# aouyang1/go-muse

Hardware: AMD Instinct MI355X
Metric: series-pairs XCorr/sec at N=4096, 1M-series batch; achieved HBM GB/s (higher is better)
Workload: dtype f64

## Files before the change

go-muse_amd/binding.py:

```python
import ctypes
import os

import numpy as np

from . import build as _build

_i32 = ctypes.c_int32
_i64 = ctypes.c_int64
_f64 = ctypes.c_double
_vp = ctypes.c_void_p
_dp = ctypes.POINTER(ctypes.c_double)
_i32p = ctypes.POINTER(ctypes.c_int32)
_i64p = ctypes.POINTER(ctypes.c_int64)

MUSE_OK = 0
MUSE_ERR_INVALID = -1
MUSE_ERR_LENGTH = -2
MUSE_ERR_ZERO_STD = -3
MUSE_ERR_NO_DEVICE = -4
MUSE_ERR_HIP = -5
MUSE_ERR_UNSUPPORTED = -6
MUSE_ERR_NOMEM = -7
MUSE_ERR_EMPTY = -8
MUSE_LAG_WINDOW_MAX = 63
# ... 116 lines not shown
                                                        _i64p, _i32p, _dp, _i32p, _dp]),
    "muse_test_many_lag_range_plan": (ctypes.c_int, [_i32, _i32, _i32, _i32, _i32, _i32p]),
    "muse_test_window_many_plan_rows": (ctypes.c_int, [_i32, _i32, _i32p, _i32p, _i32p, _i32p, _i32p, _i32p]),
    "muse_batch_run_many": (ctypes.c_int, [ctypes.POINTER(_vp), _i32, _i32p, _i32, _i32, _i32, _f64, _i32, _i32,
                                           _i64p, _i32p, _dp, _i32p, _dp]),
    "muse_batch_free": (ctypes.c_int, [_vp]),
    "muse_xcorr_with_x": (ctypes.c_int, [_vp, _dp, _dp, _i32, _i32, _dp, _i32p, _dp, _i32p]),
    "muse_xcorr": (ctypes.c_int, [_vp, _dp, _i32, _dp, _i32, _i32, _i32, _dp, _i32p, _dp, _i32p]),
    "muse_xcorr_groups": (ctypes.c_int, [_vp, _vp, _i32, _i32, _i32p, _dp, _i32p, _dp]),
    "muse_xcorr_batch": (ctypes.c_int, [_vp, _dp, _dp, _i64, _i32, _i32, _i32, _i32, _i32p, _dp, _i32p, _dp]),
    "muse_ctx_set_spectrum_cache": (ctypes.c_int, [_vp, _i32]),
    "muse_group_spectrum_cache": (ctypes.c_int, [_vp, _i64p, _i64p]),
    "muse_group_drop_spectrum_cache": (ctypes.c_int, [_vp]),
    "muse_test_spectrum_cache_limits": (ctypes.c_int, [_vp, _i64, _i64]),
    "muse_test_spectrum_cache_reader": (ctypes.c_int, [_vp, _i32]),
    "muse_test_spectrum_cache_policy": (ctypes.c_int, [_i64, _i32, _i32, _i32, _i64, _i64, _i64, _i32p, _i64p, _i64p]),
    "muse_test_batch_redo_pairs": (ctypes.c_int, [_vp, _i64p, _i64, _i64p]),
    "muse_next_pow2": (_i64, [_f64]),
}


class MuseError(RuntimeError):
    def __init__(self, status, message):
        super().__init__("muse_hip status %d: %s" % (status, message))
        self.status = status
        self.message = message


_lib = None

# ... 46 lines not shown
```

go-muse_amd/csrc/capi_batch.hip:

```cpp
#include "capi_internal.h"
#include "xcorr_huge.h"

using namespace muse;


int ilog2(int64_t n)
{
    int l = 0;
    while (((int64_t)1 << l) < n)
        l++;
    return l;
}

int build_spectrum(muse_ctx *ctx, const double *ref_host, int N, int n, int normalize, double x_scale,
                          double xc_scale, double2 *X, double2 *xc, float2 *xcf, double *xs, int *zero_std)
{
    double *dref = nullptr;
    int *dstat = nullptr;
    double2 *dscr = nullptr;
    HIP_TRY(dmalloc(ctx, &dref, (size_t)N * sizeof(double)));
    hipError_t e = dmalloc(ctx, &dstat, sizeof(int));
    if (e == hipSuccess && n > GENERIC_LDS_MAX_N)
        e = dmalloc(ctx, &dscr, (size_t)n * sizeof(double2));
    if (e == hipSuccess)
// ... 74 lines not shown
        return fail(MUSE_ERR_INVALID, "series length 1 has no sample standard deviation");
    const int64_t n = muse_next_pow2((double)N);
    if (n > HUGE_MAX_N)
        return fail(MUSE_ERR_UNSUPPORTED, "FFT length %lld > %d is not built", (long long)n, HUGE_MAX_N);
    const bool huge = n > GENERIC_MAX_N;
    muse_batch *b = new (std::nothrow) muse_batch();
    if (!b)
        return fail(MUSE_ERR_NOMEM, "host allocation failed");
    b->ctx = ctx;
    b->g = g;
    g->refs.fetch_add(1);
    ctx->refs.fetch_add(1);
    b->N = N;
    b->n = (int32_t)n;
    b->logn = ilog2(n);
    hipError_t e = dmalloc(ctx, &b->ovf_count, 2 * sizeof(int));
    if (e == hipSuccess && !huge)
        e = ensure_gscratch(ctx, n);
    muse_spectrum *sp = new (std::nothrow) muse_spectrum();
    if (!sp)
        e = hipErrorOutOfMemory;
    b->sp = sp;
    if (e == hipSuccess)
        e = dmalloc(ctx, &sp->X, (size_t)(n / 2 + 1) * sizeof(double2));
    if (huge) {
        if (e == hipSuccess)
            e = dmalloc(ctx, &sp->xcp, (size_t)n * sizeof(double2));
        if (e != hipSuccess) {
            muse_batch_free(b);
            return fail(MUSE_ERR_NOMEM, "hipMalloc failed: %s", hipGetErrorString(e));
        }
// ... 97 lines not shown
    if (rc)
        return rc;
    muse_batch *b = new (std::nothrow) muse_batch();
    if (!b)
        return fail(MUSE_ERR_NOMEM, "host allocation failed");
    b->ctx = ctx;
    b->g = g;
    g->refs.fetch_add(1);
    ctx->refs.fetch_add(1);
    b->N = src->N;
    b->n = src->n;
    b->logn = src->logn;
    b->sp = src->sp;
    b->sp->refs.fetch_add(1);
    adopt_spectrum(b);
    hipError_t e = dmalloc(ctx, &b->ovf_count, 2 * sizeof(int));
    if (e != hipSuccess) {
        muse_batch_free(b);
        return fail(MUSE_ERR_NOMEM, "hipMalloc failed: %s", hipGetErrorString(e));
    }
    *out = b;
    return MUSE_OK;
}

extern "C" int muse_batch_fft_len(muse_batch *b, int32_t *n)
{
    if (!b || !n)
        return fail(MUSE_ERR_INVALID, "NULL argument");
    *n = b->n;
    return MUSE_OK;
}
// ... 262 lines not shown
    ctx->zc_min_rows.store(min_rows < 0 ? ZC_MIN_ROWS : min_rows);
    ctx->zc_budget.store(budget_bytes < 0 ? -1 : budget_bytes);
    return MUSE_OK;
}

extern "C" int muse_test_spectrum_cache_reader(muse_ctx *ctx, int32_t reader)
{
    if (!ctx)
        return fail(MUSE_ERR_INVALID, "NULL context");
    if (reader != 0 && reader != 1)
        return fail(MUSE_ERR_INVALID, "spectrum cache reader %d (0 = two workgroups per CU, 1 = four)", (int)reader);
    ctx->zc_reader.store(reader);
    return MUSE_OK;
}

extern "C" int muse_test_spectrum_cache_policy(int64_t rows, int32_t N, int32_t f32, int32_t mode, int64_t min_rows,
                                               int64_t free_bytes, int64_t budget_bytes, int32_t *decision,
                                               int64_t *rows_cached, int64_t *bytes)
{
    if (!decision || !rows_cached || !bytes)
        return fail(MUSE_ERR_INVALID, "NULL output");
    *decision = spectrum_cache_policy(rows, N, f32 != 0, mode, min_rows < 0 ? ZC_MIN_ROWS : min_rows, free_bytes,
                                      budget_bytes < 0 ? -1 : budget_bytes, rows_cached, bytes);
    return MUSE_OK;
}

extern "C" int muse_test_batch_redo_pairs(muse_batch *b, int64_t *pairs, int64_t cap, int64_t *count)
{
    if (!b || !count || cap < 0 || (cap > 0 && !pairs))
        return fail(MUSE_ERR_INVALID, "bad redo-list arguments");
// ... 92 lines not shown
    const bool allow_spectrum_cache = pass.allow_spectrum_cache;
    const SlideFuse *slide = pass.slide;
    if (slide) {
        if (variant != KERNEL_R16_FOLD || allow_spectrum_cache)
            return fail(MUSE_ERR_INVALID, "the fused slide runs in the default n = 4096 kernel, off the rows");
        p.slide_tails = slide->tails;
        p.slide_k = slide->k;
    }
    if (variant == KERNEL_GENERIC && b->n <= GENERIC_LDS_MAX_N)
        p.gscratch = nullptr;
    LaunchTimer timer(ctx, false, st);
    LaunchTimer redo_timer(ctx, true, st);
    if (variant == KERNEL_R16_FOLD) {
        HIP_TRY(b->ovf_list.ensure(ctx, 2 * p.npairs, st));
        p.ovf_count = b->ovf_count;
        p.work_counter = b->ovf_count + 1;
        p.ovf_list = b->ovf_list.p;
        HIP_TRY(hipMemsetAsync(b->ovf_count, 0, 2 * sizeof(int), st));
        ZcPlan plan;
        std::unique_lock<std::mutex> zc_lock(b->g->ready_mu, std::defer_lock);
        if (allow_spectrum_cache && !mask && spectrum_cache_candidate(b, variant)) {
            zc_lock.lock();
            rc = plan_spectrum_cache(b, plan);
            if (rc)
                return rc;
            if (!plan.use)
                zc_lock.unlock();
        }
        HIP_TRY(timer.begin());
        if (plan.use) {
            bool launched = false;
            const auto next_launch = [&]() {
                const hipError_t e = launched ? hipMemsetAsync(b->ovf_count + 1, 0, sizeof(int), st) : hipSuccess;
                launched = true;
                return e;
            };
            const bool occ4_reader = ctx->zc_reader.load() == 1;
            for (const auto &sg : plan.readers) {
                FusedParams r = p;
                r.npairs = sg.pairs;
                HIP_TRY(next_launch());
                HIP_TRY(launch_cached(r, SpectrumCacheArgs{sg.zc(), sg.zstat(), sg.pair0, sg.pairs}, ctx->num_cus, st, occ4_reader));
            }
            if (plan.tail_pair0 < p.npairs) {
                FusedParams w = p;
                w.npairs = p.npairs - plan.tail_pair0;
                HIP_TRY(next_launch());
                HIP_TRY(launch_cache_fill(w, SpectrumCacheArgs{plan.tail_zpairs ? plan.tail_seg.zc() : nullptr,
                                                               plan.tail_zpairs ? plan.tail_seg.zstat() : nullptr,
                                                               plan.tail_pair0, plan.tail_zpairs}, ctx->num_cus, st));
            }
            zc_lock.unlock();
        } else {
            HIP_TRY(launch_fused(p, variant, ctx->num_cus, st));
        }
        HIP_TRY(timer.end());
        FusedParams q = p;
        q.slide_tails = nullptr;
        q.slide_k = 0;
        q.pair_list = b->ovf_list.p;
        q.pair_count = b->ovf_count;
        q.dense_total = ctx->variant == 0 ? p.npairs : 0;
        q.npairs = std::min<long long>(p.npairs, (long long)ctx->num_cus * 3);
        HIP_TRY(redo_timer.begin());
        HIP_TRY(launch_fused(q, KERNEL_R16_OCC3, ctx->num_cus, st));
        HIP_TRY(redo_timer.end());
        if (p.npairs >= 1024 && !(b->handoff_host && b->handoff_M == M && b->handoff_rewrites == b->g->rewrites)) {
            if (!b->handoff_host)
// ... 72 lines not shown
                 window_wide(b->g->rows, b->g->stride) ? "true" : "false");
    } else if (b->n > GENERIC_MAX_N) {
        snprintf(k, sizeof(k), "huge_rows<false>");
    } else {
        const KernelChoice kc = choose_kernel(b, (b->g->M + 1) / 2);
        switch (kc.error ? -1 : kc.variant) {
        case KERNEL_R16_FOLD: {
            bool cached = false;
            if (spectrum_cache_candidate(b, kc.variant)) {
                std::lock_guard<std::mutex> lock(b->g->ready_mu);
                int64_t rc_ = 0, by_ = 0;
                cached = b->g->zc_state == muse_group::ZC_VALID && b->g->zc_rewrites == b->g->rewrites && b->g->zc_rows > 0 &&
                         spectrum_cache_policy(b->g->M, b->N, false, b->ctx->zc_mode.load(), b->ctx->zc_min_rows.load(), 0, 0, &rc_, &by_) != ZC_POLICY_NONE;
            }
            if (cached)
                snprintf(k, sizeof(k), "xcorr_cached_n4096%s<%s>", b->ctx->zc_reader.load() == 1 ? "_occ4" : "", padded);
            else
                snprintf(k, sizeof(k), "xcorr_fused_n4096_fold<false, %s, %s>", padded, f32);
            break;
        }
        case KERNEL_R16_OCC3: snprintf(k, sizeof(k), "xcorr_fused_n4096_occ4"); break;
        case KERNEL_SMALL: snprintf(k, sizeof(k), "xcorr_fused_small<%d, %s, false, %s>", b->logn, padded, f32); break;
        case KERNEL_LONG: snprintf(k, sizeof(k), "xcorr_fused_long<%d, %s, false>", b->logn, padded); break;
        case KERNEL_STOCKHAM: snprintf(k, sizeof(k), b->n >= 8192 ? "xcorr_fused_stk_4step" : "xcorr_fused_stockham"); break;
        case KERNEL_REAL_SPLIT: snprintf(k, sizeof(k), "xcorr_fused_real32k_split<%s>", padded); break;
        case KERNEL_REAL: snprintf(k, sizeof(k), "xcorr_fused_real%dk<%s>", b->n / 1024, padded); break;
        default: break;
        }
    }
    snprintf(name, (size_t)cap, "%s", k);
    return MUSE_OK;
// ... 14 lines not shown
        dfree(c, b->sp->xcf);
        dfree(c, b->sp->xs);
        dfree(c, b->sp->c1);
        delete b->sp;
    }
    if (b->small_out) {
        std::lock_guard<std::mutex> lock(c->small_mu);
        c->small_free.emplace_back(b->small_out, b->small_cap);
    }
    dfree(c, b->ovf_count);
    hfree(c, b->handoff_host);
    hfree(c, b->refine_host);
    hfree(c, b->err_host);
    dfree(c, b->err_dev);
    b->ovf_list.release(c);
    b->mv.release(c);
    b->lag.release(c);
    b->gid_dev.release(c);
    b->gkey.release(c);
    b->gfirst.release(c);
    b->gwin.release(c);
    b->rec.release(c);
    b->selkey.release(c);
    b->cand.release(c);
    b->cnt.release(c);
    b->cand_host.release(c);
    b->cnt_host.release(c);
    b->rec_host.release(c);
    b->key_host.release(c);
    b->scr_flags.release(c);
// ... 17 lines not shown
```

go-muse_amd/csrc/capi_internal.h:

```cpp
#pragma once
#include <hip/hip_runtime.h>

#include <algorithm>
#include <atomic>
#include <mutex>
#include <cmath>
#include <cstdarg>
#include <cstdio>
#include <cstdlib>
#include <cstring>
#include <ctime>
#include <limits>
#include <map>
#include <new>
#include <string>
#include <unordered_map>
#include <utility>
#include <vector>

#include "muse_hip.h"
#include "muse_hip_test.h"
#include "xcorr_kernels.h"

using namespace muse;
// ... 92 lines not shown
    MemPool dev_pool, host_pool;
    HugeWork huge;
    int huge_batch_mb = 0;
    std::mutex huge_mu;
    std::mutex small_mu;
    std::vector<std::pair<unsigned char *, int>> small_free;
    unsigned long long small_token = 0;
    std::mutex timing_mu;
    std::atomic<bool> rows_always_copy{false};
    std::vector<void *> rows_slots;
    std::mutex rows_mu;
    std::atomic<int> zc_mode{1};
    std::atomic<int64_t> zc_min_rows{ZC_MIN_ROWS};
    std::atomic<int64_t> zc_budget{-1};
    std::atomic<int> zc_reader{0};
    std::atomic<int> win_rows_slices{0};
    std::atomic<bool> in_window_force{false};
    std::atomic<int> slide_in_window_force{0};
    std::atomic<bool> gather_nt{false};
    std::atomic<int> refs{1};
};

struct muse_group {
    std::atomic<int> refs{1};
    muse_ctx *ctx = nullptr;
    double *rows = nullptr;
    float *rows32 = nullptr;
    bool f32 = false;
    size_t elem() const { return f32 ? sizeof(float) : sizeof(double); }
    void *base() const { return f32 ? (void *)rows32 : (void *)rows; }
// ... 74 lines not shown
        OWN = 0,
        PLAIN = MUSE_IN_WINDOW_PLAIN, MFMA = MUSE_IN_WINDOW_MFMA, MASKED = MUSE_IN_WINDOW_MASKED
    };
    static constexpr int32_t MANY = -1;
    Kind kind = OWN;
    LagRange window{0, 0, 0};
    int32_t variant = 0;
    int32_t tiles = 0;
    int32_t slide = 0;
    static ScoreOrigin packed(int32_t tiles) { return ScoreOrigin{PACKED, LagRange{0, 0, 0}, 0, tiles}; }
    static ScoreOrigin in_window(int32_t path, const LagRange &w, int32_t variant = 0) { return ScoreOrigin{(Kind)path, w, variant}; }
    int32_t in_window_path() const { return kind > OWN ? (int32_t)kind : 0; }
    int32_t mfma_tiles() const { return (window.rows() + 15) / 16; }
};

struct muse_batch {
    muse_ctx *ctx = nullptr;
    muse_group *g = nullptr;
    hipStream_t own_stream = nullptr;
    hipStream_t stream() const { return own_stream ? own_stream : ctx->stream; }
    int32_t N = 0, n = 0, logn = 0;
    muse_spectrum *sp = nullptr;
    double *c1 = nullptr;
    double2 *X = nullptr, *xc = nullptr;
    double2 *xcp = nullptr;
    double2 *xcw = nullptr;
    float2 *xcf = nullptr;
    double *xs = nullptr;
    int *ovf_count = nullptr;
    int *handoff_host = nullptr;
    int64_t handoff_M = -1;
    uint64_t handoff_rewrites = 0;
    PoolBuf<long long> ovf_list;
    PoolBuf<double> mv;
    PoolBuf<int> lag;
    unsigned char *small_out = nullptr;
    int small_cap = 0;
    PoolBuf<int> gid_dev;
    std::vector<int32_t> gid_host;
    bool gid_valid = false;
    PoolBuf<unsigned long long> gkey;
    PoolBuf<long long> gfirst, gwin;
    GroupWork gw() const { return GroupWork{gkey.p, gfirst.p, gwin.p}; }
    PoolBuf<muse_record> rec;
    PoolBuf<unsigned long long> selkey;
    PoolBuf<muse_record> cand;
    PoolBuf<int> cnt;
    HostBuf<muse_record> cand_host;
// ... 181 lines not shown
```

go-muse_amd/csrc/capi_many.hip:

```cpp
#include "capi_internal.h"

using namespace muse;


int upload_many_tab(muse_ctx *ctx, std::vector<void *> &tab, bool zscratch)
{
    if (zscratch)
        HIP_TRY(ctx->zscratch.ensure(ctx, (int64_t)ctx->num_cus * 4 * 4096, ctx->stream));
    HIP_TRY(ctx->many_tab.ensure(ctx, (int64_t)tab.size(), ctx->stream));
    HIP_TRY(hipStreamSynchronize(ctx->stream));
    ctx->many_host.swap(tab);
    HIP_TRY(hipMemcpyAsync(ctx->many_tab.p, ctx->many_host.data(), ctx->many_host.size() * sizeof(void *),
                           hipMemcpyHostToDevice, ctx->stream));
    return MUSE_OK;
}

extern "C" int muse_batch_read_scores(muse_batch *b, int32_t *lag, double *mv)
{
    if (!b)
        return fail(MUSE_ERR_INVALID, "NULL batch");
    int rc = use_device(b->ctx);
    if (rc)
        return rc;
    const int64_t M = b->g->M;
// ... 85 lines not shown
    if (rc)
        return rc;
    void **const t = ctx->many_tab.p;
    FusedParams p = base_params(b0);
    p.R = R;
    p.xcp_many = (const double2 *const *)t;
    p.mv_many = (double *const *)(t + R);
    p.lag_many = (int *const *)(t + 2 * R);
    p.c1_many = (const double *const *)(t + 3 * R);
    p.zscratch = ctx->zscratch.p;
    p.zslots = (int)(ctx->zscratch.cap / 4096);
    if (mask)
        set_window(p, *mask);
    HIP_TRY(b0->ovf_list.ensure(ctx, 2 * p.npairs, b0->stream()));
    p.ovf_count = b0->ovf_count;
    p.work_counter = b0->ovf_count + 1;
    p.ovf_list = b0->ovf_list.p;
    std::unique_lock<std::mutex> scratch_lock(ctx->stage_mu, std::defer_lock);
    if (long_n || real_n) {
        scratch_lock.lock();
        p.gscratch = ctx->gscratch.p;
        p.gscratch_slices = (long long)(ctx->gscratch.cap / b0->n);
    }
    LaunchTimer timer(ctx);
    HIP_TRY(hipMemsetAsync(b0->ovf_count, 0, 2 * sizeof(int), ctx->stream));
    HIP_TRY(timer.begin());
    if (small_n) {
        HIP_TRY(launch_fused_small(p, ctx->num_cus, ctx->stream));
    } else if (real_n) {
        p.gsmall = ctx->gsmall[4];
        HIP_TRY(launch_fused_real_split(p, ctx->num_cus, ctx->stream));
    } else if (long_n)
        HIP_TRY(launch_fused_long(p, ctx->num_cus, ctx->stream));
    else
        HIP_TRY(launch_fused_multi(p, ctx->num_cus, ctx->stream));
    HIP_TRY(timer.end());
    const bool redo = !small_n && !real_n;
    LaunchTimer redo_timer(ctx, true);
    if (redo)
        HIP_TRY(redo_timer.begin());
// ... 88 lines not shown
```

go-muse_amd/csrc/capi_rows.hip:

```cpp
#include "capi_internal.h"

using namespace muse;

namespace {
constexpr size_t ROWS_GUARD = 8192;
constexpr size_t ROWS_SLOT_MIN_ELEMS = 1u << 16;
constexpr size_t ROWS_SLOT_MAX_ELEMS = 1u << 24;
constexpr size_t ROWS_ZERO_COPY_BYTES = 256u << 10;
constexpr size_t ROWS_SLOT_KEEP_ELEMS = 1u << 20;
constexpr int ROWS_SLOTS_KEPT = 16;
}

struct RowsSlot {
    muse_group g;
    muse_batch b;
    double *dev = nullptr;
    double *host = nullptr;
    double *host_dev = nullptr;
    size_t cap_elems = 0;
    SingleGroupOut *out = nullptr;
    hipEvent_t done = nullptr;
    hipStream_t stream = nullptr;
    PoolBuf<double> win_e, win_pw, win_slabs;
    uint64_t win_serial = 0;
// ... 15 lines not shown
        (void)hipStreamSynchronize(s->stream);
    dfree(ctx, s->dev);
    if (s->host)
        hfree(ctx, s->host - ROWS_GUARD);
    if (s->out)
        (void)hipHostFree(s->out);
    if (s->done)
        (void)hipEventDestroy(s->done);
    s->g.hstats.release(ctx);
    s->b.mv.release(ctx);
    s->b.lag.release(ctx);
    s->win_e.release(ctx);
    s->win_pw.release(ctx);
    s->win_slabs.release(ctx);
    s->b.ovf_list.release(ctx);
    dfree(ctx, s->b.ovf_count);
    hfree(ctx, s->b.handoff_host);
    if (s->stream)
        (void)hipStreamDestroy(s->stream);
    delete s;
}

void rows_slots_free(muse_ctx *ctx)
{
    for (void *p : ctx->rows_slots)
        slot_destroy((RowsSlot *)p);
    ctx->rows_slots.clear();
}

static int slot_reserve(RowsSlot *s, size_t elems)
// ... 38 lines not shown
        }
    }
    if (!s) {
        s = new (std::nothrow) RowsSlot();
        if (!s)
            return fail(MUSE_ERR_NOMEM, "host allocation failed");
        s->g.ctx = ctx;
        s->b.ctx = ctx;
        s->b.g = &s->g;
        hipError_t e = hipHostMalloc((void **)&s->out, sizeof(SingleGroupOut), hipHostMallocCoherent | hipHostMallocMapped);
        if (e == hipSuccess)
            e = hipEventCreateWithFlags(&s->done, hipEventDisableTiming);
        if (e == hipSuccess)
            e = hipStreamCreateWithFlags(&s->stream, hipStreamNonBlocking);
        if (e == hipSuccess)
            e = dmalloc(ctx, &s->b.ovf_count, 2 * sizeof(int));
        if (e != hipSuccess) {
            slot_destroy(s);
            return fail(MUSE_ERR_HIP, "slot set-up failed: %s", hipGetErrorString(e));
        }
    }
    int rc = slot_reserve(s, elems);
    if (rc) {
        slot_destroy(s);
        return rc;
    }
    *out = s;
    return MUSE_OK;
}

static void slot_return(muse_ctx *ctx, RowsSlot *s)
// ... 399 lines not shown
```

go-muse_amd/csrc/n4096_pair_device.h:

```cpp
#pragma once
#include "foldk_device.h"

namespace muse {

namespace foldk {

#if defined(__HIP_DEVICE_COMPILE__)
typedef d2v __attribute__((address_space(1))) *zc_out_ptr;
typedef double __attribute__((address_space(1))) *zstat_out_ptr;
typedef const double __attribute__((address_space(4))) *zstat_in_ptr;
#endif

struct PairThread {
    int t, lane, wave;
    double invN, invNm1;
};
template <bool PADDED>
__device__ __forceinline__ PairThread pair_prologue(const FusedParams &p, double2 *g2s, double *prev_row, const int rec_stride)
{
    PairThread th;
    th.t = threadIdx.x;
    th.lane = th.t & 63;
    th.wave = __builtin_amdgcn_readfirstlane(th.t >> 6);
    th.invN = PADDED ? p.invN : 1.0 / 4096.0;
// ... 123 lines not shown
    const zstat_in_ptr sp = (zstat_in_ptr)(unsigned long long)(zstat + rel * ZC_STAT);
#pragma unroll
    for (int k = 0; k < 10; k++)
        st[k] = sp[k];
#endif
}
__device__ __forceinline__ void publish_pair_stats(double *rec, const double (&st)[10], const int t, const long long rA, const bool hasB)
{
    if (t == 0) {
#pragma unroll
        for (int k = 0; k < 10; k++)
            rec[24 + k] = st[k];
        rec[34] = (double)rA;
        rec[35] = hasB ? 1.0 : 0.0;
    }
}

struct NoTap {
    static constexpr long long first = 0;
    __device__ __forceinline__ void operator()(const double2 (&)[16], const double *, double, double, long long, int) const {}
};

template <bool TIMING, bool PADDED, bool F32, bool WIN, bool SLIDE, typename Tap>
__device__ __forceinline__ void pair_loop_from_rows(const FusedParams &p, const Tap tap)
{
    __shared__ double2 xbuf[OCC_XBUF];
    __shared__ double2 g2s[128];
    __shared__ double red[2 * REC];
    __shared__ int next_s[2];
    const PairThread th = pair_prologue<PADDED>(p, g2s, red + 34, REC);
// ... 106 lines not shown
```

go-muse_amd/csrc/xcorr_kernels.h:

```cpp
#pragma once
#include <hip/hip_runtime.h>
#include <stdint.h>
#include <type_traits>

#include "muse_hip.h"

namespace muse {

enum { KERNEL_GENERIC = 0, KERNEL_R16_OCC3 = 6, KERNEL_STOCKHAM = 10, KERNEL_R16_FOLD = 11, KERNEL_SMALL = 12, KERNEL_LONG = 13, KERNEL_REAL = 14, KERNEL_REAL_SPLIT = 15 };

struct FusedParams {
    const double *rows;
    const float *rows32;
    long long M;
    long long stride;
    long long npairs;
    int N;
    int n;
    int logn;
    int normalize_y;
    const double2 *xc;
    const double2 *tw1;
    const double2 *tw2;
    const double2 *xcp;
// ... 35 lines not shown
    int scr_need_sign;
    int *ovf_count;
    int *work_counter;
    long long *ovf_list;
    const long long *pair_list;
    const int *pair_count;
    long long dense_total;
    long long gscratch_slices;
    const double *xrows;
    long long xstride;
    int Nx;
    double invN, invNm1;
    int win, win_lpos, win_lneg;
    const void *slide_tails;
    int slide_k;
};
inline FusedParams with_reciprocals(FusedParams p)
{
    p.invN = 1.0 / (double)p.N;
    p.invNm1 = 1.0 / (double)(p.N - 1);
    return p;
}
inline bool window_bounds_ok(const FusedParams &p)
{
    return !p.win || (p.win_lpos >= 0 && p.win_lneg >= 0 && p.win_lpos <= 2048 && p.win_lneg <= 2047);
}
template <typename F>
inline void with_bools(F f)
{
    f();
}
// ... 206 lines not shown
```

go-muse_amd/csrc/xcorr_r16_cached.hip:

```cpp
#include <hip/hip_runtime.h>
#include <stdint.h>
#include <algorithm>

#include "n4096_pair_device.h"

namespace muse {

struct CacheTap {
    const SpectrumCacheArgs c;
    const long long first;
    __device__ __forceinline__ void operator()(const double2 (&v)[16], const double *rec, const double s1a, const double s1b,
                                               const long long rel, const int t) const
    {
#if defined(__HIP_DEVICE_COMPILE__)
        if (rel < c.zpairs) {
            const foldk::zc_out_ptr zo = (foldk::zc_out_ptr)(unsigned long long)(c.zc + rel * 4096) + t;
#pragma unroll
            for (int i = 0; i < 16; i++)
                __builtin_nontemporal_store(occ4::d2v{v[i].x, v[i].y}, zo + 256 * i);
            if (t < 10) {
                const foldk::zstat_out_ptr so = (foldk::zstat_out_ptr)(unsigned long long)(c.zstat + rel * ZC_STAT);
                so[t] = t < 8 ? rec[24 + t] : (t == 8 ? s1a : s1b);
            }
        }
// ... 15 lines not shown
        switch (s) {
        case 0: return foldk::G3Derived::sq(foldk::G3Derived::sq(w8));
        case 1: return foldk::G3Derived::sq(w8);
        case 2: return w8;
        case 3: return make_double2(H * (w8.x + w8.y), H * (w8.y - w8.x));
        case 4: return w16;
        case 5: return foldk::G3Derived::mulc(w16, fold::C16_1, fold::S16_1);
        case 6: return make_double2(H * (w16.x + w16.y), H * (w16.y - w16.x));
        default: return foldk::G3Derived::mulc(w16, fold::S16_1, fold::C16_1);
        }
    }
};

constexpr int ZC_CLAIM = 2;

template <bool PADDED>
__global__ __launch_bounds__(OCC_THREADS, 2) void xcorr_cached_n4096(const FusedParams p, const SpectrumCacheArgs c)
{
    using namespace occ4;
    using namespace fold;
    using namespace foldk;
    __shared__ double2 xbuf[OCC_XBUF_FULL];
    __shared__ double2 g2s[128];
    __shared__ double red[2 * REC];
    __shared__ int next_s[2];
    const PairThread th = pair_prologue<PADDED>(p, g2s, red + 34, REC);
    const int t = th.t, lane = th.lane, wave = th.wave;
    const double invN = th.invN, invNm1 = th.invNm1;
    double2 *const xw = xbuf + 1088 * wave;
    const long long first = c.pair0, total = c.pair0 + p.npairs;
    constexpr bool AHEAD = !PADDED;
    constexpr int ch = ZC_CLAIM;

    if (t == 0)
        next_s[1] = (int)gridDim.x + atomicAdd(p.work_counter, 1);
    d2v zn[16];
    request_z(zn, c, first + (long long)ch * blockIdx.x, t);
    double2 xf[16];
#pragma unroll
    for (int j = 0; j < 16; j++)
        xf[j] = XcFetch{p.xcp, t}(j);
    G3Lazy g3{G3Fetch{p.g3b, t}(2), G3Fetch{p.g3b, t}(4)};
    __syncthreads();

    int parity = 0, cpar = 0;
    long long pair = first + (long long)ch * blockIdx.x;
    long long cbeg = pair, cend = pair + ch < total ? pair + ch : total;
    long long nchunk = first + (long long)ch * __builtin_amdgcn_readfirstlane(next_s[1]), after = 0;
    while (pair < total) {
        const bool claiming = pair == cbeg;
        const long long nextpair = pair + 1 < cend ? pair + 1 : nchunk;
        const long long rA = 2 * pair;
        const bool hasB = rA + 1 < p.M;
        double *const rec = red + REC * parity;
        const double *const prec = red + REC * (parity ^ 1);
        double st[10];
        load_pair_stats(st, c.zstat, pair - first);
        double2 v[16];
#pragma unroll
        for (int i = 0; i < 16; i++)
            v[i] = make_double2(zn[i].x, zn[i].y);
        xc_stage1_pre(v, xf);
        int claim = 0;
#pragma unroll
        for (int i = 0; i < 16; i += 4)
            asm volatile("" : "+v"(v[i].x), "+v"(v[i].y), "+v"(v[i + 1].x), "+v"(v[i + 1].y), "+v"(v[i + 2].x), "+v"(v[i + 2].y), "+v"(v[i + 3].x), "+v"(v[i + 3].y));
#if defined(__HIP_DEVICE_COMPILE__)
        if (claiming && t == 0) {
            unsigned long long wc = (unsigned long long)p.work_counter;
            asm volatile("" : "+v"(wc));
            claim = __hip_atomic_fetch_add((int __attribute__((address_space(1))) *)wc, 1, __ATOMIC_RELAXED, __HIP_MEMORY_SCOPE_AGENT);
        }
#endif
        const long long nxt = nextpair < total ? nextpair : first;
        if (AHEAD) {
            fence();
            request_z(zn, c, nxt, t);
            fence();
        }
        asm volatile("" : "+v"(g3.w8.x), "+v"(g3.w8.y), "+v"(g3.w16.x), "+v"(g3.w16.y));
        dft16_rn_s234(v);
        exchange_local_full<0>(v, xw, t);
        gdft16_nr(v, G2Fetch{g2s, t & 15});
        if (claiming && t == 0)
            next_s[cpar] = (int)gridDim.x + claim;
        exchange_cross_full<1, 1>(v, xbuf, t);
        lds_barrier();
        finalize_pair(prec, wave, lane == 0, invN, invNm1, p);
        publish_pair_stats(rec, st, t, rA, hasB);
        if (claiming) {
            after = first + (long long)ch * __builtin_amdgcn_readfirstlane(next_s[cpar]);
            cpar ^= 1;
        }
        gdft16_nr_l2(v, g3);
        if (PADDED)
            correct_padded<16>(v, p.c1, t, st[8] * invN, st[9] * invN, [&]() __attribute__((always_inline)) {
                request_z(zn, c, nxt, t);
                fence();
            });
        wave_argmax_store(v, wave, lane, rec + 6 * wave);
        parity ^= 1;
        if (pair + 1 < cend) {
            pair++;
        } else {
            pair = cbeg = nchunk;
            cend = pair + ch < total ? pair + ch : total;
            nchunk = after;
        }
    }
    lds_barrier();
    finalize_pair(red + REC * (parity ^ 1), t, true, invN, invNm1, p);
}

template <bool PADDED>
__global__ __launch_bounds__(OCC_THREADS, 4) void xcorr_cached_n4096_occ4(const FusedParams p, const SpectrumCacheArgs c)
{
    using namespace occ4;
    using namespace fold;
    using namespace foldk;
    __shared__ double2 xbuf[OCC_XBUF];
    __shared__ double2 g2s[128];
    __shared__ double red[2 * REC];
    __shared__ int next_s[2];
    const PairThread th = pair_prologue<PADDED>(p, g2s, red + 34, REC);
    const int t = th.t, lane = th.lane, wave = th.wave;
    const double invN = th.invN, invNm1 = th.invNm1;
// ... 50 lines not shown
}

hipError_t launch_cache_fill(const FusedParams &p_in, const SpectrumCacheArgs &c, int num_cus, hipStream_t stream)
{
    const FusedParams p = with_reciprocals(p_in);
    if (!cache_launch_ok(p, c) || c.zpairs < 0 || c.zpairs > p.npairs || (c.zpairs > 0 && (!c.zc || !c.zstat)) ||
        2 * (c.pair0 + c.zpairs) > p.M)
        return hipErrorInvalidValue;
    const dim3 g((unsigned)std::min<long long>(p.npairs, (long long)num_cus * 4)), b(OCC_THREADS);
    with_bools([&](auto padded) { hipLaunchKernelGGL((xcorr_cache_fill_n4096<decltype(padded)::value>), g, b, 0, stream, p, c); }, p.N < 4096);
    return hipGetLastError();
}

hipError_t launch_cached(const FusedParams &p_in, const SpectrumCacheArgs &c, int num_cus, hipStream_t stream, bool occ4)
{
    const FusedParams p = with_reciprocals(p_in);
    if (!cache_launch_ok(p, c) || !c.zc || !c.zstat || c.zpairs < p.npairs || 2 * (c.pair0 + p.npairs) > p.M)
        return hipErrorInvalidValue;
    const dim3 g((unsigned)(occ4 ? std::min<long long>(p.npairs, (long long)num_cus * 4)
                                 : std::min<long long>((p.npairs + ZC_CLAIM - 1) / ZC_CLAIM, (long long)num_cus * 2))), b(OCC_THREADS);
    with_bools([&](auto four, auto padded) {
        if (decltype(four)::value)
            hipLaunchKernelGGL((xcorr_cached_n4096_occ4<decltype(padded)::value>), g, b, 0, stream, p, c);
        else
            hipLaunchKernelGGL((xcorr_cached_n4096<decltype(padded)::value>), g, b, 0, stream, p, c);
    }, occ4, p.N < 4096);
    return hipGetLastError();
}

}

#undef MUSE_CONSUME_ROWS
```

go-muse_amd/muse.py:

```python
import ctypes
import math
import sys
import threading
import uuid
import weakref

import numpy as np

from . import binding as B
from .binding import MuseError

DefaultLabel = "uid"

SignFilter_POS = 1
SignFilter_NEG = -1
SignFilter_ANY = 0


class Engine:

    def __init__(self, device=0):
        self._h = ctypes.c_void_p()
        B.check(B.load().muse_ctx_create(int(device), ctypes.byref(self._h)))
        self.device = int(device)
# ... 33 lines not shown

    def set_screening(self, enable, min_rows=None):
        B.check(B.load().muse_ctx_set_screening(self._h, (int(min_rows) if min_rows and min_rows > 1 else 1) if enable else 0))

    def set_screen_bound_scale(self, scale):
        B.check(B.load().muse_test_set_screen_bound_scale(self._h, float(scale)))

    def set_spectrum_cache(self, on):
        B.check(B.load().muse_ctx_set_spectrum_cache(self._h, 1 if on else 0))

    def spectrum_cache_limits(self, min_rows=-1, budget_bytes=-1):
        B.check(B.load().muse_test_spectrum_cache_limits(self._h, int(min_rows), int(budget_bytes)))

    def spectrum_cache_reader(self, reader=0):
        B.check(B.load().muse_test_spectrum_cache_reader(self._h, int(reader)))

    def trim(self):
        B.check(B.load().muse_ctx_trim(self._h))

    def pool_stats(self):
        v = [ctypes.c_int64(0) for _ in range(4)]
        B.check(B.load().muse_test_pool_stats(self._h, *[ctypes.byref(x) for x in v]))
        return tuple(int(x.value) for x in v)

    def xcorr_repeat(self, repeat):
        B.check(B.load().muse_test_xcorr_repeat(self._h, int(repeat)))

    def huge_batch_mb(self, megabytes):
        B.check(B.load().muse_test_huge_batch_mb(self._h, int(megabytes)))

# ... 1435 lines not shown
```

Baseline: 160.5 million.

## Add sharded work-counter hand-out for cached reader and pad counter word

Adds an optional sharded pair hand-out for the cached N=4096 reader kernel. It is tunable through test hooks: several atomic counters spaced a configurable stride apart, each workgroup starting at a home shard and moving on when that shard runs out, plus a configurable claim size. The default work counter is also moved to a separate 256-byte-offset word, so it no longer shares a cache line with the overflow count. The aim is to cut atomic contention and false sharing on a single counter, at the cost of extra memsets and a more complex claim path.

```diff
diff --git a/go-muse_amd/binding.py b/go-muse_amd/binding.py
--- a/go-muse_amd/binding.py
+++ b/go-muse_amd/binding.py
@@ -154,6 +154,8 @@
     "muse_group_drop_spectrum_cache": (ctypes.c_int, [_vp]),
     "muse_test_spectrum_cache_limits": (ctypes.c_int, [_vp, _i64, _i64]),
     "muse_test_spectrum_cache_reader": (ctypes.c_int, [_vp, _i32]),
+    "muse_test_handout": (ctypes.c_int, [_vp, _i32, _i32]),
+    "muse_test_handout_stride": (ctypes.c_int, [_vp, _i32]),
     "muse_test_spectrum_cache_policy": (ctypes.c_int, [_i64, _i32, _i32, _i32, _i64, _i64, _i64, _i32p, _i64p, _i64p]),
     "muse_test_batch_redo_pairs": (ctypes.c_int, [_vp, _i64p, _i64, _i64p]),
     "muse_next_pow2": (_i64, [_f64]),
diff --git a/go-muse_amd/csrc/capi_batch.hip b/go-muse_amd/csrc/capi_batch.hip
--- a/go-muse_amd/csrc/capi_batch.hip
+++ b/go-muse_amd/csrc/capi_batch.hip
@@ -112,7 +112,7 @@
     b->N = N;
     b->n = (int32_t)n;
     b->logn = ilog2(n);
-    hipError_t e = dmalloc(ctx, &b->ovf_count, 2 * sizeof(int));
+    hipError_t e = dmalloc(ctx, &b->ovf_count, OVF_COUNT_INTS * sizeof(int));
     if (e == hipSuccess && !huge)
         e = ensure_gscratch(ctx, n);
     muse_spectrum *sp = new (std::nothrow) muse_spectrum();
@@ -240,7 +240,7 @@
     b->sp = src->sp;
     b->sp->refs.fetch_add(1);
     adopt_spectrum(b);
-    hipError_t e = dmalloc(ctx, &b->ovf_count, 2 * sizeof(int));
+    hipError_t e = dmalloc(ctx, &b->ovf_count, OVF_COUNT_INTS * sizeof(int));
     if (e != hipSuccess) {
         muse_batch_free(b);
         return fail(MUSE_ERR_NOMEM, "hipMalloc failed: %s", hipGetErrorString(e));
@@ -533,6 +533,32 @@
     return MUSE_OK;
 }
 
+extern "C" int muse_test_handout(muse_ctx *ctx, int32_t shards, int32_t claim)
+{
+    if (!ctx)
+        return fail(MUSE_ERR_INVALID, "NULL context");
+    if (shards < 0 || shards > HANDOUT_MAX_SHARDS || claim < 0 || claim > HANDOUT_MAX_CLAIM)
+        return fail(MUSE_ERR_INVALID, "pair hand-out of %d counters, %d pairs per add (0 = the default; at most %d and %d)", (int)shards,
+                    (int)claim, HANDOUT_MAX_SHARDS, HANDOUT_MAX_CLAIM);
+    ctx->hand_shards.store(shards);
+    ctx->hand_claim.store(claim);
+    return MUSE_OK;
+}
+
+extern "C" int muse_test_handout_stride(muse_ctx *ctx, int32_t bytes)
+{
+    if (!ctx)
+        return fail(MUSE_ERR_INVALID, "NULL context");
+    int shift = 0;
+    while (bytes > 0 && (4 << shift) < bytes)
+        shift++;
+    if (bytes < 0 || (bytes > 0 && ((4 << shift) != bytes || shift < 4 || shift > HANDOUT_SHIFT_MAX)))
+        return fail(MUSE_ERR_INVALID, "hand-out counters %d bytes apart (0 = the default; a power of two, 64 ... %d)", (int)bytes,
+                    4 << HANDOUT_SHIFT_MAX);
+    ctx->hand_shift.store(shift);
+    return MUSE_OK;
+}
+
 extern "C" int muse_test_spectrum_cache_policy(int64_t rows, int32_t N, int32_t f32, int32_t mode, int64_t min_rows,
                                                int64_t free_bytes, int64_t budget_bytes, int32_t *decision,
                                                int64_t *rows_cached, int64_t *bytes)
@@ -655,9 +681,25 @@
     if (variant == KERNEL_R16_FOLD) {
         HIP_TRY(b->ovf_list.ensure(ctx, 2 * p.npairs, st));
         p.ovf_count = b->ovf_count;
-        p.work_counter = b->ovf_count + 1;
         p.ovf_list = b->ovf_list.p;
-        HIP_TRY(hipMemsetAsync(b->ovf_count, 0, 2 * sizeof(int), st));
+        HIP_TRY(hipMemsetAsync(b->ovf_count, 0, (OVF_HAND_WORD + 1) * sizeof(int), st));
+        const int hook_shards = ctx->hand_shards.load(), hook_claim = ctx->hand_claim.load(), hook_shift = ctx->hand_shift.load();
+        const int shards = std::max(hook_shards, 1);
+        p.hand_shift = hook_shift ? hook_shift : HANDOUT_SHIFT;
+        p.work_counter = b->ovf_count + OVF_HAND_WORD;
+        bool fresh = true;
+        if (shards > 1) {
+            HIP_TRY(b->hand.ensure(ctx, (((int64_t)shards - 1) << p.hand_shift) + 1, st));
+            p.work_counter = b->hand.p;
+            fresh = false;
+        }
+        const auto hand_out = [&](FusedParams &f, const bool reader) {
+            f.hand_shards = reader ? hook_shards : 0;
+            f.hand_claim = reader ? hook_claim : 0;
+            const bool zeroed = fresh;
+            fresh = false;
+            return zeroed ? hipSuccess : hipMemsetAsync(p.work_counter, 0, (((size_t)(reader ? shards : 1) - 1) << p.hand_shift) * sizeof(int) + sizeof(int), st);
+        };
         ZcPlan plan;
         std::unique_lock<std::mutex> zc_lock(b->g->ready_mu, std::defer_lock);
         if (allow_spectrum_cache && !mask && spectrum_cache_candidate(b, variant)) {
@@ -670,29 +712,24 @@
         }
         HIP_TRY(timer.begin());
         if (plan.use) {
-            bool launched = false;
-            const auto next_launch = [&]() {
-                const hipError_t e = launched ? hipMemsetAsync(b->ovf_count + 1, 0, sizeof(int), st) : hipSuccess;
-                launched = true;
-                return e;
-            };
             const bool occ4_reader = ctx->zc_reader.load() == 1;
             for (const auto &sg : plan.readers) {
                 FusedParams r = p;
                 r.npairs = sg.pairs;
-                HIP_TRY(next_launch());
+                HIP_TRY(hand_out(r, true));
                 HIP_TRY(launch_cached(r, SpectrumCacheArgs{sg.zc(), sg.zstat(), sg.pair0, sg.pairs}, ctx->num_cus, st, occ4_reader));
             }
             if (plan.tail_pair0 < p.npairs) {
                 FusedParams w = p;
                 w.npairs = p.npairs - plan.tail_pair0;
-                HIP_TRY(next_launch());
+                HIP_TRY(hand_out(w, false));
                 HIP_TRY(launch_cache_fill(w, SpectrumCacheArgs{plan.tail_zpairs ? plan.tail_seg.zc() : nullptr,
                                                                plan.tail_zpairs ? plan.tail_seg.zstat() : nullptr,
                                                                plan.tail_pair0, plan.tail_zpairs}, ctx->num_cus, st));
             }
             zc_lock.unlock();
         } else {
+            HIP_TRY(hand_out(p, false));
             HIP_TRY(launch_fused(p, variant, ctx->num_cus, st));
         }
         HIP_TRY(timer.end());
@@ -795,7 +832,8 @@
                          spectrum_cache_policy(b->g->M, b->N, false, b->ctx->zc_mode.load(), b->ctx->zc_min_rows.load(), 0, 0, &rc_, &by_) != ZC_POLICY_NONE;
             }
             if (cached)
-                snprintf(k, sizeof(k), "xcorr_cached_n4096%s<%s>", b->ctx->zc_reader.load() == 1 ? "_occ4" : "", padded);
+                snprintf(k, sizeof(k), "xcorr_cached_n4096%s<%s>", b->ctx->zc_reader.load() == 1 ? "_occ4" :
+                         b->ctx->hand_shards.load() || b->ctx->hand_claim.load() ? "_sharded" : "", padded);
             else
                 snprintf(k, sizeof(k), "xcorr_fused_n4096_fold<false, %s, %s>", padded, f32);
             break;
@@ -840,6 +878,7 @@
     hfree(c, b->err_host);
     dfree(c, b->err_dev);
     b->ovf_list.release(c);
+    b->hand.release(c);
     b->mv.release(c);
     b->lag.release(c);
     b->gid_dev.release(c);
diff --git a/go-muse_amd/csrc/capi_internal.h b/go-muse_amd/csrc/capi_internal.h
--- a/go-muse_amd/csrc/capi_internal.h
+++ b/go-muse_amd/csrc/capi_internal.h
@@ -130,6 +130,7 @@
     std::atomic<int64_t> zc_min_rows{ZC_MIN_ROWS};
     std::atomic<int64_t> zc_budget{-1};
     std::atomic<int> zc_reader{0};
+    std::atomic<int> hand_shards{0}, hand_claim{0}, hand_shift{0};
     std::atomic<int> win_rows_slices{0};
     std::atomic<bool> in_window_force{false};
     std::atomic<int> slide_in_window_force{0};
@@ -234,6 +235,7 @@
     int32_t mfma_tiles() const { return (window.rows() + 15) / 16; }
 };
 
+constexpr int OVF_HAND_WORD = 64, OVF_COUNT_INTS = 128;
 struct muse_batch {
     muse_ctx *ctx = nullptr;
     muse_group *g = nullptr;
@@ -252,6 +254,7 @@
     int64_t handoff_M = -1;
     uint64_t handoff_rewrites = 0;
     PoolBuf<long long> ovf_list;
+    PoolBuf<int> hand;
     PoolBuf<double> mv;
     PoolBuf<int> lag;
     unsigned char *small_out = nullptr;
diff --git a/go-muse_amd/csrc/capi_many.hip b/go-muse_amd/csrc/capi_many.hip
--- a/go-muse_amd/csrc/capi_many.hip
+++ b/go-muse_amd/csrc/capi_many.hip
@@ -123,7 +123,7 @@
         set_window(p, *mask);
     HIP_TRY(b0->ovf_list.ensure(ctx, 2 * p.npairs, b0->stream()));
     p.ovf_count = b0->ovf_count;
-    p.work_counter = b0->ovf_count + 1;
+    p.work_counter = b0->ovf_count + OVF_HAND_WORD;
     p.ovf_list = b0->ovf_list.p;
     std::unique_lock<std::mutex> scratch_lock(ctx->stage_mu, std::defer_lock);
     if (long_n || real_n) {
@@ -132,7 +132,7 @@
         p.gscratch_slices = (long long)(ctx->gscratch.cap / b0->n);
     }
     LaunchTimer timer(ctx);
-    HIP_TRY(hipMemsetAsync(b0->ovf_count, 0, 2 * sizeof(int), ctx->stream));
+    HIP_TRY(hipMemsetAsync(b0->ovf_count, 0, (OVF_HAND_WORD + 1) * sizeof(int), ctx->stream));
     HIP_TRY(timer.begin());
     if (small_n) {
         HIP_TRY(launch_fused_small(p, ctx->num_cus, ctx->stream));
diff --git a/go-muse_amd/csrc/capi_rows.hip b/go-muse_amd/csrc/capi_rows.hip
--- a/go-muse_amd/csrc/capi_rows.hip
+++ b/go-muse_amd/csrc/capi_rows.hip
@@ -53,6 +53,7 @@
     s->win_pw.release(ctx);
     s->win_slabs.release(ctx);
     s->b.ovf_list.release(ctx);
+    s->b.hand.release(ctx);
     dfree(ctx, s->b.ovf_count);
     hfree(ctx, s->b.handoff_host);
     if (s->stream)
@@ -121,7 +122,7 @@
         if (e == hipSuccess)
             e = hipStreamCreateWithFlags(&s->stream, hipStreamNonBlocking);
         if (e == hipSuccess)
-            e = dmalloc(ctx, &s->b.ovf_count, 2 * sizeof(int));
+            e = dmalloc(ctx, &s->b.ovf_count, OVF_COUNT_INTS * sizeof(int));
         if (e != hipSuccess) {
             slot_destroy(s);
             return fail(MUSE_ERR_HIP, "slot set-up failed: %s", hipGetErrorString(e));
diff --git a/go-muse_amd/csrc/handout.h b/go-muse_amd/csrc/handout.h
--- /dev/null
+++ b/go-muse_amd/csrc/handout.h
@@ -0,0 +1,41 @@
+#pragma once
+
+#if defined(__HIPCC__) || defined(__CUDACC__)
+#define MUSE_HANDOUT_FN __host__ __device__ inline
+#else
+#define MUSE_HANDOUT_FN inline
+#endif
+
+namespace muse {
+
+constexpr int HANDOUT_MAX_SHARDS = 256;
+constexpr int HANDOUT_MAX_CLAIM = 4;
+
+MUSE_HANDOUT_FN long long handout_chunks(const long long npairs, const int ch)
+{
+    return (npairs + ch - 1) / ch;
+}
+
+MUSE_HANDOUT_FN int handout_chunk(const int shard, const int ticket, const int S, const int C, const int grid)
+{
+    const unsigned D = (unsigned)(C - grid), q = D / (unsigned)S, r = D - q * (unsigned)S;
+    const unsigned s = (unsigned)shard;
+    const unsigned lo = s * q + (s < r ? s : r), len = q + (s < r ? 1u : 0u);
+    return (unsigned)ticket < len ? grid + (int)(lo + (unsigned)ticket) : -1;
+}
+
+MUSE_HANDOUT_FN int handout_begin(const int home)
+{
+    return home;
+}
+MUSE_HANDOUT_FN int handout_shard(const int state)
+{
+    return state & 511;
+}
+MUSE_HANDOUT_FN int handout_used_up(const int state, const int S)
+{
+    const int shard = handout_shard(state), found = (state >> 9) + 1;
+    return found >= S ? -1 : (found << 9) | (shard + 1 == S ? 0 : shard + 1);
+}
+
+}
diff --git a/go-muse_amd/csrc/n4096_pair_device.h b/go-muse_amd/csrc/n4096_pair_device.h
--- a/go-muse_amd/csrc/n4096_pair_device.h
+++ b/go-muse_amd/csrc/n4096_pair_device.h
@@ -161,6 +161,32 @@
         rec[34] = (double)rA;
         rec[35] = hasB ? 1.0 : 0.0;
     }
+}
+
+__device__ __forceinline__ int handout_home(const FusedParams &p)
+{
+    return handout_begin(__builtin_amdgcn_readfirstlane((int)(blockIdx.x % (unsigned)p.hand_shards)));
+}
+__device__ __forceinline__ int2 claim_chunk(const FusedParams &p, int state, int ticket, bool drawn)
+{
+    int chunk = -1;
+    while (state >= 0) {
+        const int shard = handout_shard(state);
+        if (!drawn)
+            ticket = atomicAdd(p.work_counter + ((long long)shard << p.hand_shift), 1);
+        drawn = false;
+        chunk = handout_chunk(shard, ticket, p.hand_shards, p.hand_chunks, (int)gridDim.x);
+        if (chunk >= 0)
+            break;
+        state = handout_used_up(state, p.hand_shards);
+    }
+    return make_int2(chunk >= 0 ? chunk : p.hand_chunks, state);
+}
+__device__ __forceinline__ void take_claim(const int2 *slot, int &chunk, int &state)
+{
+    const int2 c = *slot;
+    chunk = __builtin_amdgcn_readfirstlane(c.x);
+    state = __builtin_amdgcn_readfirstlane(c.y);
 }
 
 struct NoTap {
diff --git a/go-muse_amd/csrc/xcorr_kernels.h b/go-muse_amd/csrc/xcorr_kernels.h
--- a/go-muse_amd/csrc/xcorr_kernels.h
+++ b/go-muse_amd/csrc/xcorr_kernels.h
@@ -3,6 +3,7 @@
 #include <stdint.h>
 #include <type_traits>
 
+#include "handout.h"
 #include "muse_hip.h"
 
 namespace muse {
@@ -73,7 +74,23 @@
     int win, win_lpos, win_lneg;
     const void *slide_tails;
     int slide_k;
-};
+    int hand_shards, hand_claim, hand_shift;
+    int hand_chunks;
+};
+constexpr int HANDOUT_SHIFT = 6;
+constexpr int HANDOUT_SHIFT_MAX = 10;
+inline bool handout_resolve(FusedParams &p, const int default_claim)
+{
+    if (p.hand_shards == 0)
+        p.hand_shards = 1;
+    if (p.hand_claim == 0)
+        p.hand_claim = default_claim;
+    if (p.hand_shards < 1 || p.hand_shards > HANDOUT_MAX_SHARDS || p.hand_claim < 1 || p.hand_claim > HANDOUT_MAX_CLAIM ||
+        p.hand_shift < 0 || p.hand_shift > HANDOUT_SHIFT_MAX || p.npairs < 1 || p.npairs > 0x7fffffff - (1 << 20))
+        return false;
+    p.hand_chunks = (int)handout_chunks(p.npairs, p.hand_claim);
+    return true;
+}
 inline FusedParams with_reciprocals(FusedParams p)
 {
     p.invN = 1.0 / (double)p.N;
diff --git a/go-muse_amd/csrc/xcorr_r16_cached.hip b/go-muse_amd/csrc/xcorr_r16_cached.hip
--- a/go-muse_amd/csrc/xcorr_r16_cached.hip
+++ b/go-muse_amd/csrc/xcorr_r16_cached.hip
@@ -53,8 +53,8 @@
 
 constexpr int ZC_CLAIM = 2;
 
-template <bool PADDED>
-__global__ __launch_bounds__(OCC_THREADS, 2) void xcorr_cached_n4096(const FusedParams p, const SpectrumCacheArgs c)
+template <bool PADDED, bool SHARDED>
+__device__ __forceinline__ void cached_reader(const FusedParams &p, const SpectrumCacheArgs &c)
 {
     using namespace occ4;
     using namespace fold;
@@ -62,17 +62,22 @@
     __shared__ double2 xbuf[OCC_XBUF_FULL];
     __shared__ double2 g2s[128];
     __shared__ double red[2 * REC];
-    __shared__ int next_s[2];
+    __shared__ int2 next_s[2];
     const PairThread th = pair_prologue<PADDED>(p, g2s, red + 34, REC);
     const int t = th.t, lane = th.lane, wave = th.wave;
     const double invN = th.invN, invNm1 = th.invNm1;
     double2 *const xw = xbuf + 1088 * wave;
     const long long first = c.pair0, total = c.pair0 + p.npairs;
     constexpr bool AHEAD = !PADDED;
-    constexpr int ch = ZC_CLAIM;
-
-    if (t == 0)
-        next_s[1] = (int)gridDim.x + atomicAdd(p.work_counter, 1);
+    const int ch = SHARDED ? p.hand_claim : ZC_CLAIM;
+
+    const int home = SHARDED ? handout_home(p) : 0;
+    if (t == 0) {
+        if (SHARDED)
+            next_s[1] = claim_chunk(p, home, 0, false);
+        else
+            next_s[1].x = (int)gridDim.x + atomicAdd(p.work_counter, 1);
+    }
     d2v zn[16];
     request_z(zn, c, first + (long long)ch * blockIdx.x, t);
     double2 xf[16];
@@ -85,7 +90,12 @@
     int parity = 0, cpar = 0;
     long long pair = first + (long long)ch * blockIdx.x;
     long long cbeg = pair, cend = pair + ch < total ? pair + ch : total;
-    long long nchunk = first + (long long)ch * __builtin_amdgcn_readfirstlane(next_s[1]), after = 0;
+    int shard = 0, k;
+    if (SHARDED)
+        take_claim(next_s + 1, k, shard);
+    else
+        k = __builtin_amdgcn_readfirstlane(next_s[1].x);
+    long long nchunk = first + (long long)ch * k, after = 0;
     while (pair < total) {
         const bool claiming = pair == cbeg;
         const long long nextpair = pair + 1 < cend ? pair + 1 : nchunk;
@@ -105,8 +115,8 @@
         for (int i = 0; i < 16; i += 4)
             asm volatile("" : "+v"(v[i].x), "+v"(v[i].y), "+v"(v[i + 1].x), "+v"(v[i + 1].y), "+v"(v[i + 2].x), "+v"(v[i + 2].y), "+v"(v[i + 3].x), "+v"(v[i + 3].y));
 #if defined(__HIP_DEVICE_COMPILE__)
-        if (claiming && t == 0) {
-            unsigned long long wc = (unsigned long long)p.work_counter;
+        if (claiming && t == 0 && (!SHARDED || shard >= 0)) {
+            unsigned long long wc = (unsigned long long)(SHARDED ? p.work_counter + ((long long)handout_shard(shard) << p.hand_shift) : p.work_counter);
             asm volatile("" : "+v"(wc));
             claim = __hip_atomic_fetch_add((int __attribute__((address_space(1))) *)wc, 1, __ATOMIC_RELAXED, __HIP_MEMORY_SCOPE_AGENT);
         }
@@ -121,14 +131,22 @@
         dft16_rn_s234(v);
         exchange_local_full<0>(v, xw, t);
         gdft16_nr(v, G2Fetch{g2s, t & 15});
-        if (claiming && t == 0)
-            next_s[cpar] = (int)gridDim.x + claim;
+        if (claiming && t == 0) {
+            if (SHARDED)
+                next_s[cpar] = claim_chunk(p, shard, claim, true);
+            else
+                next_s[cpar].x = (int)gridDim.x + claim;
+        }
         exchange_cross_full<1, 1>(v, xbuf, t);
         lds_barrier();
         finalize_pair(prec, wave, lane == 0, invN, invNm1, p);
         publish_pair_stats(rec, st, t, rA, hasB);
         if (claiming) {
-            after = first + (long long)ch * __builtin_amdgcn_readfirstlane(next_s[cpar]);
+            if (SHARDED)
+                take_claim(next_s + cpar, k, shard);
+            else
+                k = __builtin_amdgcn_readfirstlane(next_s[cpar].x);
+            after = first + (long long)ch * k;
             cpar ^= 1;
         }
         gdft16_nr_l2(v, g3);
@@ -149,6 +167,17 @@
     }
     lds_barrier();
     finalize_pair(red + REC * (parity ^ 1), t, true, invN, invNm1, p);
+}
+
+template <bool PADDED>
+__global__ __launch_bounds__(OCC_THREADS, 2) void xcorr_cached_n4096(const FusedParams p, const SpectrumCacheArgs c)
+{
+    cached_reader<PADDED, false>(p, c);
+}
+template <bool PADDED>
+__global__ __launch_bounds__(OCC_THREADS, 2) void xcorr_cached_n4096_sharded(const FusedParams p, const SpectrumCacheArgs c)
+{
+    cached_reader<PADDED, true>(p, c);
 }
 
 template <bool PADDED>
@@ -229,17 +258,21 @@
 
 hipError_t launch_cached(const FusedParams &p_in, const SpectrumCacheArgs &c, int num_cus, hipStream_t stream, bool occ4)
 {
-    const FusedParams p = with_reciprocals(p_in);
-    if (!cache_launch_ok(p, c) || !c.zc || !c.zstat || c.zpairs < p.npairs || 2 * (c.pair0 + p.npairs) > p.M)
+    FusedParams p = with_reciprocals(p_in);
+    const bool sharded = !occ4 && (p.hand_shards != 0 || p.hand_claim != 0);
+    if (!cache_launch_ok(p, c) || !c.zc || !c.zstat || c.zpairs < p.npairs || 2 * (c.pair0 + p.npairs) > p.M ||
+        (sharded && !handout_resolve(p, ZC_CLAIM)))
         return hipErrorInvalidValue;
     const dim3 g((unsigned)(occ4 ? std::min<long long>(p.npairs, (long long)num_cus * 4)
-                                 : std::min<long long>((p.npairs + ZC_CLAIM - 1) / ZC_CLAIM, (long long)num_cus * 2))), b(OCC_THREADS);
-    with_bools([&](auto four, auto padded) {
+                                 : std::min<long long>(sharded ? p.hand_chunks : (p.npairs + ZC_CLAIM - 1) / ZC_CLAIM, (long long)num_cus * 2))), b(OCC_THREADS);
+    with_bools([&](auto four, auto shards, auto padded) {
         if (decltype(four)::value)
             hipLaunchKernelGGL((xcorr_cached_n4096_occ4<decltype(padded)::value>), g, b, 0, stream, p, c);
+        else if (decltype(shards)::value)
+            hipLaunchKernelGGL((xcorr_cached_n4096_sharded<decltype(padded)::value>), g, b, 0, stream, p, c);
         else
             hipLaunchKernelGGL((xcorr_cached_n4096<decltype(padded)::value>), g, b, 0, stream, p, c);
-    }, occ4, p.N < 4096);
+    }, occ4, sharded, p.N < 4096);
     return hipGetLastError();
 }
 
diff --git a/go-muse_amd/muse.py b/go-muse_amd/muse.py
--- a/go-muse_amd/muse.py
+++ b/go-muse_amd/muse.py
@@ -71,6 +71,11 @@
 
     def spectrum_cache_reader(self, reader=0):
         B.check(B.load().muse_test_spectrum_cache_reader(self._h, int(reader)))
+
+    def handout(self, shards=0, claim=0, stride=None):
+        B.check(B.load().muse_test_handout(self._h, int(shards), int(claim)))
+        if stride is not None:
+            B.check(B.load().muse_test_handout_stride(self._h, int(stride)))
 
     def trim(self):
         B.check(B.load().muse_ctx_trim(self._h))
```

New measurement: 160.5 million, median of 2. No clear change (+0.0%).
